# Shridhar2602/WebGPU-Path-Tracer

Hardware: AMD Instinct MI355X
Metric: Mrays/s at 1080p, 8 bounces; achieved HBM GB/s vs roofline (higher is better)
Workload: dtype f32; 1 GPU; configs[1]: Cornell + monkey_968.obj (967 tris), 1920x1080, 64 spp, 8 bounces, stack_size 20; parallelism=1 GPU

## Files before the change

webgpu-path-tracer_amd/csrc/ptmi.hip:

```cpp
#include <dlfcn.h>
#include <hip/hip_runtime.h>
#include <rccl/rccl.h>

#include <algorithm>
#include <chrono>
#include <cmath>
#include <cstdio>
#include <cstdlib>
#include <condition_variable>
#include <cstring>
#include <functional>
#include <map>
#include <memory>
#include <mutex>
#include <string>
#include <thread>
#include <type_traits>
#include <vector>

#include "../../include/ptmi.h"
#include "ptmi_dbuf.h"
#include "ptmi_kernels.h"
#include "ptmi_denoise_kernels.h"
#include "ptmi_tuning.h"
// ... 705 lines not shown
    HIP_TRY(c, hipEventRecord(ev.e0, c->stream));
    if (int r = dry()) return r;
    HIP_TRY(c, hipEventRecord(ev.e1, c->stream));
    HIP_TRY(c, hipEventSynchronize(ev.e1));
    HIP_TRY(c, hipEventElapsedTime(ms, ev.e0, ev.e1));
    return PTMI_OK;
  };
  float best = 0.0f;
  if (int r = score(&best)) return r;
  uint64_t sets = 1;
  if (c->tun.debug_placement) fprintf(stderr, "ptmi placement: set 0 %.3f ms\n", best);
  DBuf* mine[10] = {&c->d_q0[0], &c->d_q0[1], &c->d_q1[0], &c->d_q1[1], &c->d_q2[0], &c->d_q2[1], &c->d_tp[0], &c->d_tp[1], &c->d_hm[0], &c->d_hm[1]};
  const size_t width[10] = {16, 16, 16, 16, 16, 16, 8, 8, 4, 4};
  int rc_out = PTMI_OK;
  std::vector<DBuf> losers;
  size_t set_bytes = 0;
  for (int k = 0; k < 10; k++) set_bytes += slots * width[k];
  for (int t = 1; t < c->tun.placement_tries; t++) {
    size_t mem_free = 0, mem_total = 0;
    if (hipMemGetInfo(&mem_free, &mem_total) != hipSuccess) mem_free = 0, (void)hipGetLastError();
    if (mem_free < set_bytes + ((size_t)8 << 30)) {
      if (losers.empty()) break;
      losers.clear();
    }
    DBuf cand[10];
    bool ok = true;
    for (int k = 0; k < 10 && ok; k++) ok = cand[k].ensure(slots * width[k]) == hipSuccess;
    float ms = 0.0f;
    if (ok) {
      for (int k = 0; k < 10; k++) std::swap(*mine[k], cand[k]);
      rc_out = score(&ms);
      ok = rc_out == PTMI_OK;
      if (ok) sets++;
      if (c->tun.debug_placement) fprintf(stderr, "ptmi placement: set %d %.3f ms\n", t, ms);
      if (!ok || ms >= best) {
        for (int k = 0; k < 10; k++) std::swap(*mine[k], cand[k]);
      } else {
        best = ms;
      }
    }
    if (!ok) {
      (void)hipStreamSynchronize(c->stream);
      break;
    }
    for (DBuf& b : cand)
      if (b.p) losers.push_back(std::move(b));
  }
  restore.stats.placement_sets = sets;
  restore.stats.placement_ms = std::chrono::duration<double, std::milli>(std::chrono::steady_clock::now() - t_search).count();
  return rc_out;
}

RenderConst make_render_const(const ptmi_ctx* c, const float* view16, uint32_t frame0, int n_frames, int reset_first) {
  const ptmi_params& p = c->prm;
  RenderConst rc{};
  rc.W = (float)c->W;
  rc.H = (float)c->H;
  memcpy(rc.view, view16, 64);
  {
    const float* m = rc.view;
    for (int k = 0; k < 3; k++) rc.cam_o[k] = ((m[k] * 0.0f + m[4 + k] * 0.0f) + m[8 + k] * 0.0f) + m[12 + k] * 1.0f;
  }
  rc.fov_factor = (float)(1.0 / std::tan((double)p.fov_degrees * (3.14159265358979323846 / 180.0) / 2.0));
  rc.bg[0] = p.background[0], rc.bg[1] = p.background[1], rc.bg[2] = p.background[2];
  rc.max_bounces = p.max_bounces;
  rc.stratify = p.stratify ? 1 : 0;
  if (p.stratify) {
    float sqrt_spp = (float)std::sqrt((double)p.num_samples);
    int side = 0;
    for (float i = 0.0f; i < sqrt_spp; i += 1.0f) side++;
    rc.strat_side = side;
    rc.recip_sqrt_spp = 1.0f / (float)(int)sqrt_spp;
    rc.num_samples = side * side;
    rc.sample_div = (float)(side * side);
  } else {
    rc.strat_side = 1;
    rc.recip_sqrt_spp = 1.0f;
    rc.num_samples = p.num_samples;
    rc.sample_div = (float)p.num_samples;
  }
  rc.stack_size = p.stack_size;
  rc.light_mix = p.light_mix;
  rc.surface_mix = 1.0f - p.light_mix;
  rc.npix = (uint32_t)c->W * (uint32_t)c->H;
  rc.frame0 = frame0;
  rc.n_frames = n_frames;
  rc.reset_first = reset_first;
  rc.rank = c->rank, rc.world = c->world, rc.tile = c->tile;
  rc.n_local = count_local(rc.npix, c->rank, c->world, c->tile);
  rc.shade_cont = (uint32_t)c->tun.shade_cont;
  return rc;
}

struct ViewBatch {
  ViewTab vt;
  float4* stack;
};

int render_batch(ptmi_ctx* c, const float* view16, uint32_t frame0, int n_frames, int reset_first, int fold = -1, int dry_steps = 0, const ViewBatch* views = nullptr) {
  const ptmi_params& p = c->prm;
  c->ahead.valid = false;
  const RenderConst rc = make_render_const(c, view16, frame0, n_frames, reset_first);
  if (rc.n_local == 0) return PTMI_OK;
  ViewTab vtab{};
  if (views) vtab = views->vt, vtab.n_local = rc.n_local;
  const ViewTab* vt = views ? &vtab : nullptr;

  const int n_steps = rc.num_samples * p.max_bounces;
  const size_t npaths = (size_t)rc.n_local * (size_t)n_frames;
  c->batch_enqueued = false;
  int rcode = ensure_paths(c, npaths, n_steps + 2, rc.num_samples > 1);
  if (rcode) return rcode;
  StepCtl* ctl = c->d_ctl.as<StepCtl>();
  const uint32_t total = rc.n_local * (uint32_t)n_frames;
  const int sa_carry = stack_alloc_for(c);
  const bool carry = c->tun.bvh_carry > 0 && c->S.n_nodes > 0 && c->bvh_depth >= c->tun.bvh_carry_min_depth && total >= (uint32_t)c->tun.bvh_carry_min_paths && p.max_bounces > 1;
  const uint32_t resv = carry ? (uint32_t)c->tun.bvh_carry_slots : 0u;
  const int rec_words = carry_rec_words(sa_carry);
  if (carry)
    for (int k = 0; k < 2; k++) HIP_TRY(c, c->d_carry[k].ensure((size_t)resv * (size_t)rec_words * 4));
  auto carry_of = [&](int s) {
    Carry cy{};
    cy.resv = s == 0 ? 0u : resv;
    cy.resv_next = resv;
    cy.after = c->tun.bvh_carry;
    cy.rec_words = rec_words;
    cy.pool_in = c->d_carry[s & 1].as<uint32_t>();
    cy.pool_out = c->d_carry[(s + 1) & 1].as<uint32_t>();
    return cy;
  };
  const uint32_t bound = total + total / 8 + (uint32_t)c->num_cus * 8 * 1024 + resv;
  const uint32_t ew_grid = std::max<uint32_t>(1, std::min<uint32_t>((total + kBlock - 1) / kBlock, (uint32_t)c->num_cus * 16));
  const int sort_env = c->tun.sort;
  const bool sort = sort_env >= 0 ? sort_env != 0 : c->material_classes > 1;

  const auto shade = with_flags([](auto is, auto so, auto cn, auto mu) { return shade_kernel<is, so, cn, mu>(); }, p.importance_sampling != 0, sort, c->counters,
                                rc.num_samples > 1);
  const auto shade_views = with_flags([](auto is, auto so, auto cn, auto mu) { return shade_views_kernel<is, so, cn, mu>(); }, p.importance_sampling != 0, sort, c->counters,
                                      rc.num_samples > 1);
  int shade_bpc = c->tun.shade_blocks_per_cu;
  if (shade_bpc <= 0) {
    int& cached = c->shade_blocks_per_cu[views ? reinterpret_cast<const void*>(shade_views) : reinterpret_cast<const void*>(shade)];
    if (cached == 0) {
      int nb = 0;
      const hipError_t oe = views ? hipOccupancyMaxActiveBlocksPerMultiprocessor(&nb, shade_views, kBlock, 0) : hipOccupancyMaxActiveBlocksPerMultiprocessor(&nb, shade, kBlock, 0);
      if (oe != hipSuccess || nb < 1) nb = 5;
      cached = nb;
    }
    shade_bpc = cached;
  }
  const uint32_t sgrid = std::max<uint32_t>(1, std::min<uint32_t>((bound + kSChunk - 1) / kSChunk, (uint32_t)c->num_cus * (uint32_t)std::min(8, std::max(1, shade_bpc))));
  unsigned long long* tot = c->d_totals.as<unsigned long long>();
  const TailPlan tail = tail_plan(c, rc);

  if (dry_steps == 0 && c->placement_pending) {
    c->placement_pending = false;
    if (total > tail.limit_first) {
      int r = placement_search(c, [&]() { return render_batch(c, view16, frame0, n_frames, reset_first, fold, 2, views); });
      if (r) return r;
    }
  }
  ScopedSpan whole(c, T_RENDER);
  c->batch_enqueued = true;
  hipLaunchKernelGGL(k_init_ctl, dim3((unsigned)((n_steps + 2 + 63) / 64)), dim3(64), 0, c->stream, ctl, n_steps + 2, resv);
  HIP_TRY(c, hipMemsetAsync(tot + 16, 0, kTotalsBytes - 128, c->stream));
  {
    ScopedSpan s(c, T_GENERATE);
    if (rc.num_samples == 1) HIP_TRY(c, hipMemsetAsync(c->d_touched.p, 0, npaths, c->stream));
    if (views) {
      const auto generate = with_flags([](auto cn) { return &k_generate_views<cn>; }, c->counters);
      hipLaunchKernelGGL(generate, dim3(ew_grid), dim3(kBlock), 0, c->stream, c->S, rc, paths_of(c, 0, rc.num_samples > 1), ctl, c->d_heads.as<uint32_t>(), tot, vtab);
    } else {
      const auto generate = with_flags([](auto cn) { return &k_generate<cn>; }, c->counters);
      hipLaunchKernelGGL(generate, dim3(ew_grid), dim3(kBlock), 0, c->stream, c->S, rc, paths_of(c, 0, rc.num_samples > 1), ctl, c->d_heads.as<uint32_t>(), tot);
    }
    HIP_TRY(c, hipGetLastError());
    c->stats.generate_launches++;
  }
  bool drained = false;
  const int run_steps = dry_steps > 0 ? std::min(n_steps, dry_steps) : n_steps;
  for (int s = 0; s < run_steps; s++) {
    if (s >= 12 && (s & 7) == 4) {
      uint32_t left = 1;
      uint32_t rec3[3] = {1, 0, 0};
      HIP_TRY(c, hipMemcpyAsync(rec3, &ctl[s].n_rays, sizeof rec3, hipMemcpyDeviceToHost, c->stream));
      HIP_TRY(c, hipStreamSynchronize(c->stream));
      left = (rec3[0] <= resv && rec3[2] == 0) ? 0u : 1u;
      if (left == 0) {
        drained = true;
        break;
      }
    }
    Paths P = paths_of(c, s, rc.num_samples > 1);
    if (const uint32_t tail_limit = dry_steps > 0 ? 0u : (s == 0 ? tail.limit_first : tail.limit_later)) {
      int lr = launch_tail(c, rc, P, ctl + s, s == 0 ? 1 : 0, tail_limit, tail.six, carry_of(s), vt);
      if (lr) return lr;
      if (s == 0 && total <= tail_limit) {
        drained = true;
        break;
      }
    }
    if (dry_steps == 0) {
      Carry cy = carry_of(s);
      if (!carry || s >= n_steps - c->tun.bvh_carry_last) cy.resv_next = 0u;
      int lr = launch_intersect(c, P, ctl + s, bound, false, s == 0 ? &rc : nullptr, cy, vt);
      if (lr) return lr;
    }
    {
      ScopedSpan sp(c, T_SHADE);
      if (views) hipLaunchKernelGGL(shade_views, dim3(sgrid), dim3(kBlock), 0, c->stream, c->S, rc, P, ctl + s, c->d_heads.as<uint32_t>(), tot, s == 0 ? 1 : 0, s == 0 ? 0u : resv, vtab);
      else hipLaunchKernelGGL(shade, dim3(sgrid), dim3(kBlock), 0, c->stream, c->S, rc, P, ctl + s, c->d_heads.as<uint32_t>(), tot, s == 0 ? 1 : 0, s == 0 ? 0u : resv);
      HIP_TRY(c, hipGetLastError());
    }
    c->stats.intersect_launches++;
    c->stats.shade_launches++;
  }
  if (dry_steps > 0) return PTMI_OK;
  if (carry && !drained && n_steps > 0) {
    int lr = launch_tail(c, rc, paths_of(c, n_steps, rc.num_samples > 1), ctl + n_steps, 0, 0xffffffffu, tail.six, carry_of(n_steps), vt);
    if (lr) return lr;
  }
  {
    ScopedSpan s(c, T_ACCUM);
    const int f_end = fold < 0 ? n_frames : std::min(fold, n_frames);
    if (views) hipLaunchKernelGGL(k_accumulate<true>, dim3(ew_grid), dim3(kBlock), 0, c->stream, rc, paths_of(c, 0, rc.num_samples > 1), views->stack, n_steps, tot, 0, f_end, vtab);
    else hipLaunchKernelGGL(k_accumulate<false>, dim3(ew_grid), dim3(kBlock), 0, c->stream, rc, paths_of(c, 0, rc.num_samples > 1), c->fb, n_steps, tot, 0, f_end, vtab);
    c->stats.accumulate_launches++;
  }
  HIP_TRY(c, hipGetLastError());
  c->stats.frames += (uint64_t)n_frames;
  c->ahead.rc = rc;
  c->ahead.grid = ew_grid;
  return PTMI_OK;
}

int check_queue_overflow(ptmi_ctx* c) {
  if (!c->d_totals.p) return PTMI_OK;
  unsigned long long flag = 0;
  HIP_TRY(c, hipMemcpy(&flag, c->d_totals.as<unsigned long long>() + 15, sizeof flag, hipMemcpyDeviceToHost));
  if (flag) return fail(c, PTMI_ERR_STATE, "internal: a step's queue outgrew its buffer (paths were dropped); the framebuffer is incomplete");
  return PTMI_OK;
}

int check_renderable(ptmi_ctx* c) {
  if (!c->fb || c->W <= 0) return fail(c, PTMI_ERR_STATE, "no framebuffer: call ptmi_resize first");
  const ptmi_params& p = c->prm;
  if (p.importance_sampling && c->has_unknown_material)
    return fail(c, PTMI_ERR_UNSUPPORTED,
                "importance_sampling with a material_type outside {0,1,2,3}: the shader would read stale private state (scatterRec)");
  return PTMI_OK;
}

struct Rccl {
  void* lib = nullptr;
  decltype(&ncclCommInitAll) CommInitAll = nullptr;
  decltype(&ncclCommDestroy) CommDestroy = nullptr;
  decltype(&ncclCommAbort) CommAbort = nullptr;
  decltype(&ncclReduce) Reduce = nullptr;
  decltype(&ncclGroupStart) GroupStart = nullptr;
  decltype(&ncclGroupEnd) GroupEnd = nullptr;
  decltype(&ncclGetErrorString) GetErrorString = nullptr;
  std::string why;
  bool load() {
    if (lib) return true;
    const char* names[] = {getenv("PTMI_RCCL_LIB"), "librccl.so.1", "librccl.so", "/opt/rocm/lib/librccl.so.1"};
    for (const char* n : names) {
      if (!n || !*n) continue;
      lib = dlopen(n, RTLD_NOW | RTLD_LOCAL);
      if (lib) break;
      why = dlerror();
    }
    if (!lib) return false;
#define PTMI_RCCL_SYM(field, sym)                                  \
  field = reinterpret_cast<decltype(field)>(dlsym(lib, #sym));     \
  if (!field) {                                                    \
    why = std::string("librccl lacks ") + #sym;                    \
    dlclose(lib);                                                  \
    lib = nullptr;                                                 \
    return false;                                                  \
  }
    PTMI_RCCL_SYM(CommInitAll, ncclCommInitAll)
    PTMI_RCCL_SYM(CommDestroy, ncclCommDestroy)
    PTMI_RCCL_SYM(CommAbort, ncclCommAbort)
    PTMI_RCCL_SYM(Reduce, ncclReduce)
    PTMI_RCCL_SYM(GroupStart, ncclGroupStart)
    PTMI_RCCL_SYM(GroupEnd, ncclGroupEnd)
    PTMI_RCCL_SYM(GetErrorString, ncclGetErrorString)
#undef PTMI_RCCL_SYM
    return true;
  }
};
Rccl g_rccl;
inline int rccl_fail_hook(const ptmi_ctx* c) {
#ifdef PTMI_TEST_HOOKS
  return c->test_rccl_fail;
#else
  (void)c;
  return 0;
#endif
}
std::once_flag g_rccl_once;
bool rccl_loaded() {
  std::call_once(g_rccl_once, [] { (void)g_rccl.load(); });
  return g_rccl.lib != nullptr;
}

#define RCCL_TRY(c, expr)                                                                                            \
  do {                                                                                                               \
    ncclResult_t _r = (expr);                                                                                        \
    if (_r != ncclSuccess) return fail((c), PTMI_ERR_DEVICE, std::string(#expr) + ": " + g_rccl.GetErrorString(_r)); \
  } while (0)

template <class F>
int on_all_devices(ptmi_ctx* c, F fn, bool parallel = false) {
  const std::vector<ptmi_ctx*> devs = local_devices(c);
  std::vector<int> rcs(devs.size(), PTMI_OK);
  if (parallel) {
    for (ptmi_ctx* q : c->peers) {
      if (!q->worker) q->worker = std::make_unique<PeerWorker>();
      q->worker->post([&fn, q] { return fn(q); });
    }
    rcs[0] = fn(c);
    for (size_t i = 1; i < devs.size(); i++) rcs[i] = devs[i]->worker->wait();
  } else {
    for (size_t i = 0; i < devs.size(); i++)
      if ((rcs[i] = fn(devs[i]))) break;
  }
  for (size_t i = 1; i < devs.size(); i++)
    if (rcs[i] && !rcs[0]) {
      c->err = "local device #" + std::to_string(i) + " (GPU " + std::to_string(devs[i]->device) + "): " + devs[i]->err;
      return rcs[i];
    }
  return rcs[0];
}

__global__ __launch_bounds__(kBlock) void k_gather_tiles(float4* __restrict__ dst, const float4* __restrict__ src, uint32_t n_local, int rank, int world, int tile) {
  for (uint32_t j = blockIdx.x * kBlock + threadIdx.x; j < n_local; j += gridDim.x * kBlock) {
    const uint32_t tl = j / (uint32_t)tile, within = j - tl * (uint32_t)tile;
    const uint32_t pix = (tl * (uint32_t)world + (uint32_t)rank) * (uint32_t)tile + within;
    dst[pix] = src[pix];
  }
}

__global__ __launch_bounds__(kBlock) void k_add_into(float4* __restrict__ dst, const float4* __restrict__ src, size_t n) {
  for (size_t i = (size_t)blockIdx.x * kBlock + threadIdx.x; i < n; i += (size_t)gridDim.x * kBlock) {
    const float4 a = dst[i], b = src[i];
    dst[i] = make_float4(a.x + b.x, a.y + b.y, a.z + b.z, a.w + b.w);
// ... 1327 lines not shown
```

webgpu-path-tracer_amd/csrc/ptmi_kernels.h:

```cpp
#pragma once
#include "ptmi_device.h"
#include "ptmi_tuning.h"

namespace ptmi {

constexpr int kBlock = 256;

DEV void reset_heads(uint32_t* __restrict__ heads) {
  if (blockIdx.x == 0 && threadIdx.x < kMaxTeams) heads[threadIdx.x * kHeadStride] = 0u;
}

DEV void reduce_counters(const Counters& cn, unsigned long long* __restrict__ totals, bool bvh) {
  uint32_t v[5] = {cn.node_visits, cn.tri_tests, cn.sphere_tests, cn.quad_tests, cn.mat_fetches};
#pragma unroll
  for (int k = 0; k < 5; k++) {
    unsigned long long x = v[k];
    for (int off2 = 32; off2 > 0; off2 >>= 1) x += __shfl_down(x, off2, 64);
    if (lane_id() == 0 && x) {
      atomicAdd(&totals[2 + k], x);
      if (bvh && k == 0) atomicAdd(&totals[7], x);
      if (bvh && k == 4) atomicAdd(&totals[8], x);
    }
  }
}
// ... 477 lines not shown
        float pdf = rc.light_mix * lpdf + rc.surface_mix * lambertian_pdf;
        if (pdf <= 0.00001f) {
          drop_acc = true;
          sample_done = true;
        } else {
          T = T * ((lambertian_pdf * mix3(m.color, m.spec, doSpecular)) / pdf);
          no = so;
          nd = sd;
        }
      }
    } else {
      T = T * mix3(m.color, m.spec, doSpecular);
      no = sorg;
      nd = sdir;
    }
    if (!sample_done) {
      if (roulette && bounce > 2) {
        LT(LT_RR);
        float p = ptm_max(T.x, ptm_max(T.y, T.z));
        if (rand2D(rng) > p) {
          sample_done = true;
        } else {
          T = T * rcp_exact(p);
        }
      }
      if (!sample_done) {
        bounce++;
        if (bounce >= rc.max_bounces) sample_done = true;
      }
    }
  }

  const bool changes = !(add.x == 0.0f && add.y == 0.0f && add.z == 0.0f);
  ns.pid = pid;
  if (!sample_done) {
    if (changes) {
      LT(LT_ACC_CONT);
      float4 A4 = acc_load(P, pid, acc_written);
      f3 acc = mk3(A4) + add;
      acc_store(P, pid, make_float4(acc.x, acc.y, acc.z, A4.w), acc_written);
      acc_written = true;
    }
    ns.o = no, ns.d = nd, ns.T = T, ns.bounce = bounce | (acc_written ? kAccWritten : 0), ns.rng = rng;
    return true;
  }

  LT(LT_END_SAMPLE);
  if (!MULTI) {
    if (drop_acc) {
      f3 fin = mk3(0, 0, 0) + add;
      acc_store(P, pid, make_float4(fin.x, fin.y, fin.z, __int_as_float(1)), acc_written);
    } else {
      end_sample_progressive(P, pid, add, acc_written);
    }
    return false;
  } else {
  float4 A4 = P.acc[pid];
  int sample = __float_as_int(A4.w);
  f3 radiance = drop_acc ? add : (mk3(A4) + add);
  f3 sum = mk3(P.pixsum[pid]) + radiance;
  sample++;
  if (sample < rc.num_samples) {
    P.pixsum[pid] = make_float4(sum.x, sum.y, sum.z, 0.0f);
    if (MV) camera_ray_view(rc, vt, pid, sample, rng, no, nd);
    else camera_ray(rc, local_to_pixel(rc, pid % rc.n_local), sample, rng, no, nd);
    P.acc[pid] = make_float4(0.0f, 0.0f, 0.0f, __int_as_float(sample));
    ns.o = no, ns.d = nd, ns.T = mk3(1.0f, 1.0f, 1.0f), ns.bounce = 0, ns.rng = rng;
    return true;
  }
  f3 fin = sum / rc.sample_div;
  P.acc[pid] = make_float4(fin.x, fin.y, fin.z, __int_as_float(sample));
  return false;
  }
}

constexpr uint32_t kRegionDiv = 16;
constexpr uint32_t kRegionDivCont = 64;
constexpr int kTailLimitFirst = 2 << 20, kTailLimitLater = 1 << 20;
constexpr int kTailLimitFirstShallow = 24 << 20, kTailLimitLaterShallow = 2 << 20;
constexpr int kTailLimitFirstDeep = 6 << 20;
constexpr int kTailRefill = 16;
constexpr bool kMissShortcut = true;
constexpr int kSChunk = 512;

constexpr uint32_t kR0Empty = 0xffffffffu, kR0Busy = 0xfffffffeu, kR0Full = 0xfffffffdu;
__shared__ uint32_t s_region0;
constexpr uint32_t kNoSlot = 0xffffffffu;
struct OutRegion {
  uint32_t cur, rend;
  DEV uint32_t place(bool keep, uint32_t region, uint32_t wregion, uint32_t wregion_later, StepCtl* __restrict__ ctl, uint32_t cap, unsigned long long* __restrict__ totals) {
    const int lane = lane_id();
    const uint64_t km = __ballot(keep);
    const uint32_t kept = (uint32_t)__popcll(km), rank = lanes_below(km);
    const uint32_t b0 = cur, n0 = min(kept, rend - cur);
    uint32_t b1 = kNoSlot;
    cur += n0;
    if (kept > n0) {
      uint32_t nb = 0, claimed = wregion;
      bool full;
      if (rend == 0u) {
        if (lane == 0) nb = atomicCAS(&s_region0, kR0Empty, kR0Busy);
        nb = (uint32_t)__builtin_amdgcn_readfirstlane((int)nb);
        if (nb == kR0Empty) {
          if (lane == 0) {
            nb = atomicAdd(&ctl[1].n_rays, region);
            if (nb + region > cap) {
              atomicAdd(&totals[15], 1ull);
              atomicSub(&ctl[1].n_rays, region);
              nb = kR0Full;
            }
            atomicExch(&s_region0, nb);
          }
          nb = (uint32_t)__builtin_amdgcn_readfirstlane((int)nb);
        } else {
          while (nb == kR0Busy) {
            __builtin_amdgcn_s_sleep(8);
            if (lane == 0) nb = atomicAdd(&s_region0, 0u);
            nb = (uint32_t)__builtin_amdgcn_readfirstlane((int)nb);
          }
        }
        full = nb == kR0Full;
        nb += (threadIdx.x >> 6) * wregion;
      } else {
        claimed = wregion_later;
        if (lane == 0) nb = atomicAdd(&ctl[1].n_rays, claimed);
        nb = (uint32_t)__builtin_amdgcn_readfirstlane((int)nb);
        full = nb + claimed > cap;
        if (full && lane == 0) {
          atomicAdd(&totals[15], 1ull);
          atomicSub(&ctl[1].n_rays, claimed);
        }
      }
      if (!full) {
        b1 = nb;
        cur = nb + (kept - n0);
        rend = nb + claimed;
      }
    }
    if (keep && (rank < n0 || b1 != kNoSlot)) return (rank < n0) ? (b0 + rank) : (b1 + (rank - n0));
    return kNoSlot;
  }
  DEV void close(const Paths& P, uint32_t wregion, bool block_claim) {
    if (rend == 0u && block_claim && s_region0 < kR0Full) {
      cur = s_region0 + (threadIdx.x >> 6) * wregion;
      rend = cur + wregion;
    }
    for (uint32_t i = cur + (uint32_t)lane_id(); i < rend; i += 64u) {
      LT(LT_HOLE);
      mark_hole(P.out, P.hout, i);
    }
  }
};

template <bool IS, bool COUNT, bool MULTI, bool MV>
DEV void shade_body(const DevScene& S, const RenderConst& rc, const Paths& P, StepCtl* __restrict__ ctl, uint32_t* __restrict__ heads, unsigned long long* __restrict__ totals,
                    int first, uint32_t resv, const ViewTab& vt) {
  reset_heads(heads);
  __shared__ float4 s_q0[kSChunk], s_q1[kSChunk], s_q2[kSChunk];
  __shared__ uint16_t s_sorted[kSChunk];
  __shared__ uint32_t s_cnt[NUM_BINS + 2];
  __shared__ uint32_t s_nout, s_next;
  const QuadL L = load_light(S);
  const int lane = lane_id();
  const QueueExtent qe = queue_extent(ctl, resv);
  const uint32_t n = qe.n, n_carried = qe.n_carried;
  const uint32_t region = max((uint32_t)kSChunk, ((n / gridDim.x / kRegionDiv) + 511u) & ~511u);
  const uint32_t wregion = region / (kBlock / 64);
  OutRegion out = {0u, 0u};
  if (threadIdx.x == 0) s_region0 = kR0Empty;
  uint32_t my_valid = 0;
  uint32_t my_missed = 0;
  Counters cn = {0, 0, 0, 0, 0};
  auto stage = [&](bool survive, const NewState& ns) {
    const uint64_t mk = __ballot(survive);
    if (mk) {
      const int leader = __ffsll((unsigned long long)mk) - 1;
      uint32_t bb = 0;
      if (lane == leader) bb = atomicAdd(&s_nout, (uint32_t)__popcll(mk));
      bb = (uint32_t)__shfl((int)bb, leader, 64);
      if (survive) {
        const uint32_t q = bb + lanes_below(mk);
        s_q0[q] = pack_q0(ns);
        s_q1[q] = pack_q1(ns);
        s_q2[q] = pack_q2(ns);
      }
    }
  };
  for (uint32_t base = blockIdx.x * (uint32_t)kSChunk; base < n; base += gridDim.x * (uint32_t)kSChunk) {
    const uint32_t m = min((uint32_t)kSChunk, n - base);
    if (threadIdx.x < NUM_BINS) s_cnt[threadIdx.x] = 0;
    if (threadIdx.x == 0) {
      s_nout = 0;
      s_next = 0;
    }
    __syncthreads();
    {
      uint32_t keys[kSChunk / kBlock];
      uint32_t words[kSChunk / kBlock];
  #pragma unroll
      for (int r = 0; r < kSChunk / kBlock; r++) words[r] = P.hin.mat[base + min((uint32_t)r * kBlock + threadIdx.x, m - 1u)];
  #pragma unroll
      for (int r = 0; r < kSChunk / kBlock; r++) {
        const uint32_t j = (uint32_t)r * kBlock + threadIdx.x;
        int bin = -1;
        if (j < m && !dead_slot(base + j, n_carried, resv)) {
          const uint32_t b = (words[r] >> HITMAT_BIN_SHIFT) & 7u;
          if (b < (uint32_t)NUM_BINS) bin = (int)b;
        }
        uint32_t rank = 0;
        if ((uint32_t)r * kBlock < m) rank = bin_rank(bin, s_cnt);
        keys[r] = (bin < 0) ? 0xffffffffu : ((uint32_t)bin | (rank << 3));
      }
      __syncthreads();
      uint32_t nvalid = 0;
      {
        uint32_t off[NUM_BINS];
  #pragma unroll
        for (int b = 0; b < NUM_BINS; b++) {
          off[b] = nvalid;
          nvalid += s_cnt[b];
        }
  #pragma unroll
        for (int r = 0; r < kSChunk / kBlock; r++) {
          if (keys[r] != 0xffffffffu) {
            const uint32_t b = keys[r] & 7u;
            uint32_t o = off[0];
  #pragma unroll
            for (int k = 1; k < NUM_BINS; k++) o = (b == (uint32_t)k) ? off[k] : o;
            s_sorted[o + (keys[r] >> 3)] = (uint16_t)((uint32_t)r * kBlock + threadIdx.x);
          }
        }
      }
      if (threadIdx.x == 0) my_valid += nvalid;
      __syncthreads();
#pragma unroll 1
      for (;;) {
        uint32_t k0 = 0;
        if (lane == 0) k0 = atomicAdd(&s_next, 64u);
        k0 = (uint32_t)__builtin_amdgcn_readfirstlane((int)k0);
        if (k0 >= nvalid) break;
        const uint32_t k = k0 + lane;
        bool survive = false;
        NewState ns = zero_state();
        if (k < nvalid) {
          const SlotState st = load_slot<MV>(P, base + s_sorted[k], first != 0, rc, vt);
          const TriFetch tf = tri_fetch(S, P.uv, st.slot, __float_as_uint(st.tp.y));
          survive = shade_one<IS, MULTI, MV>(S, rc, P, st, tf, L, ns, vt);
        }
        stage(survive, ns);
      }
    }
    __syncthreads();
    const uint32_t cnt = s_nout;
    uint32_t missed = 0;
#pragma unroll 1
    for (uint32_t q0 = (threadIdx.x & ~63u); q0 < cnt; q0 += kBlock) {
      const uint32_t q = q0 + (uint32_t)lane;
      bool keep = false;
      float2 tp = make_float2(0.0f, 0.0f);
      uint32_t hm = 0u, rng = 0u;
      if (q < cnt) {
        const float4 a0 = s_q0[q], a1 = s_q1[q];
        rng = __float_as_uint(a0.w);
        prims_for_ray<COUNT>(S, mk3(a0), mk3(a1), rng, tp, hm, cn);
        if (kMissShortcut && !MULTI && hm == HITMAT_MISS) {
          const float4 a2 = s_q2[q];
          end_sample_progressive(P, __float_as_uint(a1.w), mk3(rc.bg[0], rc.bg[1], rc.bg[2]) * mk3(a2), (__float_as_int(a2.w) & kAccWritten) != 0);
          missed++;
        } else {
          keep = true;
        }
      }
      if (__ballot(keep) == 0ull) continue;
      const uint32_t dst = out.place(keep, region, wregion, wregion, ctl, P.cap, totals);
      if (dst != kNoSlot) {
        float4 a0 = s_q0[q];
        a0.w = __uint_as_float(rng);
        store_slot(P.out, P.hout, dst, a0, s_q1[q], s_q2[q], tp, hm);
      }
    }
    if (!MULTI) {
      for (int off2 = 32; off2 > 0; off2 >>= 1) missed += __shfl_down(missed, off2, 64);
      if (lane == 0) my_missed += missed;
    }
    __syncthreads();
  }
  if (lane == 0 && my_missed + my_valid) atomicAdd(tally_line(totals, blockIdx.x), my_missed + my_valid);
  out.close(P, wregion, blockIdx.x * (uint32_t)kSChunk < n);
  if (COUNT) reduce_counters(cn, totals, false);
}

template <bool IS, bool COUNT, bool MULTI, bool MV>
DEV void shade_body_wave(const DevScene& S, const RenderConst& rc, const Paths& P, StepCtl* __restrict__ ctl, uint32_t* __restrict__ heads,
                         unsigned long long* __restrict__ totals, int first, uint32_t resv, const ViewTab& vt) {
  reset_heads(heads);
  constexpr uint32_t kRing = 128, kWaves = kBlock / 64;
  static_assert((size_t)kWaves * kRing == (size_t)kSChunk, "the rings take the LDS the block version's staging arrays take");
  __shared__ float4 s_q0[kWaves * kRing], s_q1[kWaves * kRing], s_q2[kWaves * kRing];
  if (threadIdx.x == 0) s_region0 = kR0Empty;
#ifdef PTMI_LANE_TALLY
  if (threadIdx.x < kLaneTallies * 2) s_lane_tally[threadIdx.x] = 0u;
  if (threadIdx.x < 4 * kTimeTallies) s_time_tally[threadIdx.x] = 0ull;
  if (threadIdx.x < 4) s_time_last[threadIdx.x] = 0ull;
#endif
  __syncthreads();
  const QuadL L = load_light(S);
  const int lane = lane_id();
  const uint32_t wv = threadIdx.x >> 6;
  float4 *const r0 = s_q0 + wv * kRing, *const r1 = s_q1 + wv * kRing, *const r2 = s_q2 + wv * kRing;
  const QueueExtent qe = queue_extent(ctl, resv);
  const uint32_t n = qe.n, n_carried = qe.n_carried;
  const uint32_t cont_min = MULTI ? 0u : rc.shade_cont;
  const uint32_t region_full = max((uint32_t)kSChunk, ((n / gridDim.x / kRegionDiv) + 511u) & ~511u);
  const uint32_t region = cont_min ? max((uint32_t)kSChunk, ((n / gridDim.x / kRegionDivCont) + 511u) & ~511u) : region_full;
  const uint32_t wregion = region / kWaves, wregion_full = region_full / kWaves;
  bool pred = true;
  OutRegion out = {0u, 0u};
  uint32_t head = 0, cnt = 0;
  uint32_t my_valid = 0, my_missed = 0;
  Counters cn = {0, 0, 0, 0, 0};
  auto flush_pass = [&](uint32_t take, SlotState& cs, bool cont) {
    const uint32_t q = (head + (uint32_t)lane) & (kRing - 1u);
    bool keep = false;
    float2 tp = make_float2(0.0f, 0.0f);
    uint32_t hm = 0u, rng = 0u;
    if ((uint32_t)lane < take) {
      LT(LT_FLUSH);
      const float4 a0 = r0[q], a1 = r1[q];
      TT(TT_RING_READ, a0.x + a1.x);
      rng = __float_as_uint(a0.w);
      prims_for_ray<COUNT>(S, mk3(a0), mk3(a1), rng, tp, hm, cn);
      TT(TT_FLUSH_PRIMS, tp.x + __uint_as_float(hm));
      if (kMissShortcut && !MULTI && hm == HITMAT_MISS) {
        LT(LT_MISS_SHORTCUT);
        const float4 a2 = r2[q];
        end_sample_progressive(P, __float_as_uint(a1.w), mk3(rc.bg[0], rc.bg[1], rc.bg[2]) * mk3(a2), (__float_as_int(a2.w) & kAccWritten) != 0);
      } else {
        keep = true;
      }
    }
    bool go = false;
    if (cont_min) {
      const bool final_hit = keep && (hm & HITMAT_BVH) == 0u;
      pred = (uint32_t)__popcll(__ballot(final_hit)) >= cont_min;
      if (cont && pred) {
        go = final_hit;
        keep = keep && !final_hit;
      }
    }
    const uint64_t km = __ballot(keep);
    const uint32_t kept = (uint32_t)__popcll(km);
    my_missed += take - kept - (uint32_t)__popcll(__ballot(go));
    if (kept) {
      const uint32_t dst = out.place(keep, region, wregion, pred ? wregion : wregion_full, ctl, P.cap, totals);
      if (dst != kNoSlot) {
        LT(LT_KEEP);
        float4 a0 = r0[q];
        a0.w = __uint_as_float(rng);
        store_slot(P.out, P.hout, dst, a0, r1[q], r2[q], tp, hm);
      }
    }
    if (cont) {
      if (go) LT(LT_CONT);
      cs.q0 = r0[q];
      cs.q0.w = __uint_as_float(rng);
      cs.q1 = r1[q];
      cs.q2 = r2[q];
      cs.tp = tp;
      cs.hitmat = hm;
      cs.slot = 0u;
    }
    head = (head + take) & (kRing - 1u);
    cnt -= take;
    TT(TT_FLUSH_STORE, 0.0f);
    return go;
  };
  auto shade_group = [&](bool active, const SlotState& st) {
    bool survive = false, valid = false;
    NewState ns = zero_state();
    TT(TT_OTHER, 0.0f);
    if (active) {
      LT(LT_GROUP);
      TT(TT_LOAD1, st.q0.x + st.q1.x + st.q2.x + st.tp.x + __uint_as_float(st.hitmat));
      valid = __float_as_uint(st.q1.w) != PID_HOLE;
      if (valid) {
        LT(LT_VALID);
        const TriFetch tf = tri_fetch(S, P.uv, st.slot, __float_as_uint(st.tp.y));
        survive = shade_one<IS, MULTI, MV>(S, rc, P, st, tf, L, ns, vt);
      }
    }
    TT(TT_SHADE, ns.o.x + ns.T.x);
    my_valid += (uint32_t)__popcll(__ballot(valid));
    const uint64_t mk = __ballot(survive);
    if (survive) {
      LT(LT_STAGE);
      const uint32_t q = (head + cnt + lanes_below(mk)) & (kRing - 1u);
      r0[q] = pack_q0(ns);
      r1[q] = pack_q1(ns);
      r2[q] = pack_q2(ns);
    }
    cnt += (uint32_t)__popcll(mk);
    TT(TT_STAGE, 0.0f);
  };
  {
    uint32_t base = blockIdx.x * (uint32_t)kSChunk, j0 = wv * 64u;
    auto settle = [&]() {
      while (base < n && j0 >= min((uint32_t)kSChunk, n - base)) {
        base += gridDim.x * (uint32_t)kSChunk;
        j0 = wv * 64u;
      }
      return base < n;
    };
    auto fetch = [&](SlotState& st) {
      const uint32_t j = j0 + (uint32_t)lane;
      const bool act = j < min((uint32_t)kSChunk, n - base) && !dead_slot(base + j, n_carried, resv);
      if (act) st = load_slot<MV>(P, base + j, first != 0, rc, vt);
      return act;
    };
    SlotState cur;
    bool have = settle(), cur_act = false, again = false;
    if (have) cur_act = fetch(cur);
#pragma unroll 1
    while (have || again) {
      shade_group(cur_act, cur);
      if (!again) {
        j0 += kBlock;
        have = settle();
      }
      const bool flush_due = cnt >= 64u;
      const bool pre = have && !(cont_min && flush_due && pred);
      SlotState nxt;
      bool nxt_act = false;
      if (pre) nxt_act = fetch(nxt);
      bool go = false;
      if (flush_due) go = flush_pass(64u, nxt, cont_min != 0u && !pre);
      again = __ballot(go) != 0ull;
      if (again) nxt_act = go;
      else if (have && !pre) nxt_act = fetch(nxt);
      cur = nxt;
      cur_act = nxt_act;
    }
    if (cnt) flush_pass(cnt, cur, false);
  }
  if (MULTI) my_missed = 0;
  if (lane == 0 && my_missed + my_valid) atomicAdd(tally_line(totals, blockIdx.x), my_missed + my_valid);
  __syncthreads();
#ifdef PTMI_LANE_TALLY
  if (threadIdx.x < kLaneTallies * 2 && s_lane_tally[threadIdx.x]) atomicAdd(&g_lane_tally[threadIdx.x], (unsigned long long)s_lane_tally[threadIdx.x]);
  if (threadIdx.x < kTimeTallies) {
    unsigned long long t = 0;
    for (int w = 0; w < 4; w++) t += s_time_tally[w * kTimeTallies + threadIdx.x];
    if (t) atomicAdd(&g_time_tally[threadIdx.x], t);
  }
#endif
  out.close(P, wregion, true);
#ifdef PTMI_LANE_TALLY
  __syncthreads();
  if (threadIdx.x >= 2 * LT_HOLE && threadIdx.x < 2 * LT_HOLE + 2 && s_lane_tally[threadIdx.x]) atomicAdd(&g_lane_tally[threadIdx.x], (unsigned long long)s_lane_tally[threadIdx.x]);
#endif
  if (COUNT) reduce_counters(cn, totals, false);
}

template <bool IS, bool SORT, bool COUNT, bool MULTI>
__global__ __launch_bounds__(kBlock) PTMI_SHADE_ATTR void k_shade(DevScene S, RenderConst rc, Paths P, StepCtl* __restrict__ ctl, uint32_t* __restrict__ heads,
                                                                  unsigned long long* __restrict__ totals, int first, uint32_t resv) {
  if constexpr (SORT) shade_body<IS, COUNT, MULTI, false>(S, rc, P, ctl, heads, totals, first, resv, ViewTab{});
  else shade_body_wave<IS, COUNT, MULTI, false>(S, rc, P, ctl, heads, totals, first, resv, ViewTab{});
}
template <bool SORT, bool COUNT>
__global__ __launch_bounds__(kBlock) __attribute__((amdgpu_waves_per_eu(6, 8))) void k_shade6(DevScene S, RenderConst rc, Paths P, StepCtl* __restrict__ ctl,
                                                                                                uint32_t* __restrict__ heads, unsigned long long* __restrict__ totals, int first, uint32_t resv) {
  if constexpr (SORT) shade_body<false, COUNT, false, false>(S, rc, P, ctl, heads, totals, first, resv, ViewTab{});
  else shade_body_wave<false, COUNT, false, false>(S, rc, P, ctl, heads, totals, first, resv, ViewTab{});
}
template <bool IS, bool SORT, bool COUNT, bool MULTI>
__global__ __launch_bounds__(kBlock) PTMI_SHADE_ATTR void k_shade_views(DevScene S, RenderConst rc, Paths P, StepCtl* __restrict__ ctl, uint32_t* __restrict__ heads,
                                                                        unsigned long long* __restrict__ totals, int first, uint32_t resv, ViewTab vt) {
  if constexpr (SORT) shade_body<IS, COUNT, MULTI, true>(S, rc, P, ctl, heads, totals, first, resv, vt);
  else shade_body_wave<IS, COUNT, MULTI, true>(S, rc, P, ctl, heads, totals, first, resv, vt);
}
template <bool SORT, bool COUNT>
__global__ __launch_bounds__(kBlock) __attribute__((amdgpu_waves_per_eu(6, 8))) void k_shade6_views(DevScene S, RenderConst rc, Paths P, StepCtl* __restrict__ ctl,
                                                                                                      uint32_t* __restrict__ heads, unsigned long long* __restrict__ totals, int first,
                                                                                                      uint32_t resv, ViewTab vt) {
  if constexpr (SORT) shade_body<false, COUNT, false, true>(S, rc, P, ctl, heads, totals, first, resv, vt);
  else shade_body_wave<false, COUNT, false, true>(S, rc, P, ctl, heads, totals, first, resv, vt);
}

constexpr int kTailTravBatch = 24;
template <bool IS, bool COUNT, bool MULTI, bool NOABORT, bool MV>
DEV void tail_body(const DevScene& S, const RenderConst& rc, const Paths& P, StepCtl* __restrict__ ctl, unsigned long long* __restrict__ totals, int first, uint32_t limit,
                   int stack_size, int lds_entries, int spill_entries, int2* __restrict__ spill, const Carry& cy, const ViewTab& vt) {
  const QueueExtent qe = queue_extent(ctl, cy.resv);
  const uint32_t n = qe.n, n_carried = qe.n_carried;
  if (n == 0u) return;
  if ((n > cy.resv ? n - cy.resv : 0u) + n_carried > limit) return;
  extern __shared__ int lds_stack[];
  const int lane = lane_id();
  LaneStack2 stk;
  stk.lds = (lds_v2i_t*)lds_stack + lane;
  stk.spill = spill + (size_t)blockIdx.x * (size_t)spill_entries * 64 + lane;
  stk.lds_entries = lds_entries;
  const QuadL L = load_light(S);
  Counters cn = {0, 0, 0, 0, 0}, cb = {0, 0, 0, 0, 0};
  uint32_t tally = 0;
  const uint32_t root = __float_as_uint(S.root_lo.w);
  const uint32_t root_node = (root & REF_LEAF) ? root : (root & REF_IDX);
  SlotState st;
  st.q0 = st.q1 = st.q2 = make_float4(0.0f, 0.0f, 0.0f, 0.0f);
  st.tp = make_float2(0.0f, 0.0f);
  st.hitmat = HITMAT_HOLE, st.slot = 0;
  bool alive = false;
  bool resume = false;
  int park_sp = -1;
  float2 uv = make_float2(0.0f, 0.0f);
  uint32_t gnext = blockIdx.x, gbase = 0, pos = 64;
  Stopwatch sw;
  sw.begin();
#pragma unroll 1
  for (;;) {
    BT(TB_VOTE, 0.0f, 0);
    uint64_t am = __ballot(alive);
    const uint32_t nidle = 64u - (uint32_t)__popcll(am);
    if (nidle >= (uint32_t)kTailRefill || am == 0ull) {
      if (pos == 64u && gnext * 64u < n) {
        gbase = gnext * 64u;
        gnext += gridDim.x;
        pos = 0;
      }
      if (pos < 64u) {
        const uint32_t take = min(nidle, 64u - pos), rank = lanes_below(~am);
        if (!alive && rank < take) {
          const uint32_t slot = gbase + pos + rank;
          if (slot < n && !dead_slot(slot, n_carried, cy.resv)) {
            st = load_slot<MV>(P, slot, first != 0, rc, vt);
            alive = __float_as_uint(st.q1.w) != PID_HOLE;
            uv = make_float2(0.0f, 0.0f);
            resume = alive && slot < cy.resv;
          }
        }
        pos += take;
        am = __ballot(alive);
        BT(TB_TAKE, st.q1.x + st.tp.x + __uint_as_float(st.hitmat), take);
      }
    }
    if (am == 0ull) {
      if (pos == 64u && gnext * 64u >= n) break;
      continue;
    }
    {
      const bool flagged = alive && (st.hitmat & HITMAT_BVH) != 0u;
      const uint64_t fmask = __ballot(flagged);
      const bool more_to_take = !(pos == 64u && gnext * 64u >= n);
      if (fmask != 0ull && ((int)__popcll(fmask) >= (more_to_take ? kTailTravBatch : 1) || __ballot(alive && !flagged) == 0ull)) {
        Walk w = {flagged ? root_node : N_DONE, 0, st.tp.x, {0.0f, 0.0f, 0u, 0u}};
        WalkRay ray = make_walk_ray(S, mk3(st.q0), mk3(st.q1));
        if (flagged && resume) carry_restore(cy, st.slot, stk, w);
        resume = false;
        if (flagged && park_sp >= 0) {
          unpark(stk, park_sp, w);
          park_sp = -1;
        }
#pragma unroll 1
        for (;;) {
          const uint64_t wm = __ballot(w.node != N_DONE);
          if (wm == 0ull) break;
          if (cy.park_below > 0 && (int)__popcll(wm) < cy.park_below && (more_to_take || __ballot(alive && !(flagged && w.node != N_DONE)) != 0ull)) break;
          if ((int)w.node < 0) {
            walk_leaf<COUNT>(S, ray, stk, w, cb, sw);
            BT(TB_WALK_LEAF, w.ct, __popcll(__ballot(1)));
          }
          if (w.node < N_INNER_LIMIT) walk_inner<COUNT, NOABORT, TB_WALK_FETCH>(S, ray, stk, w, stack_size, cb, sw);
          BT(TB_WALK_STEP, __uint_as_float(w.node), __popcll(__ballot(w.node != N_DONE)));
        }
        if (flagged && w.node != N_DONE) {
          park(stk, w);
          park_sp = w.sp;
        } else {
          if (w.hit.prim != 0u) {
            st.tp = make_float2(w.ct, __uint_as_float(w.hit.prim));
            uv = make_float2(w.hit.u, w.hit.v);
            st.hitmat = w.hit.mat;
          }
          st.hitmat &= ~HITMAT_BVH;
        }
      }
      const bool go = alive && (st.hitmat & HITMAT_BVH) == 0u;
      NewState ns = zero_state();
      bool survive = false;
      if (go) {
        tally++;
        const TriFetch tf = tri_fetch_uv(S, uv, __float_as_uint(st.tp.y));
        survive = shade_one<IS, MULTI, MV>(S, rc, P, st, tf, L, ns, vt);
        alive = survive;
      }
      BT(TB_SHADE, ns.o.x + ns.T.x, __popcll(__ballot(go)));
      if (go && alive) {
        uint32_t hm;
        float2 tp;
        prims_for_ray<COUNT>(S, ns.o, ns.d, ns.rng, tp, hm, cn);
        if (kMissShortcut && !MULTI && hm == HITMAT_MISS) {
          end_sample_progressive(P, ns.pid, mk3(rc.bg[0], rc.bg[1], rc.bg[2]) * ns.T, (ns.bounce & kAccWritten) != 0);
          tally++;
          alive = false;
        } else {
          st.q0 = pack_q0(ns);
          st.q1 = pack_q1(ns);
          st.q2 = pack_q2(ns);
          st.tp = tp;
          st.hitmat = hm;
        }
      }
      BT(TB_PRIMS, st.tp.x, __popcll(__ballot(go && survive)));
    }
  }
  BT_FLUSH(g_tail_tally);
  for (int off2 = 32; off2 > 0; off2 >>= 1) tally += __shfl_down(tally, off2, 64);
  if (lane == 0 && tally) atomicAdd(tally_line(totals, blockIdx.x), tally);
  if (COUNT) {
    reduce_counters(cn, totals, false);
    reduce_counters(cb, totals, true);
  }
  if (lane == 0) {
    __threadfence();
    if (atomicAdd(&ctl->tail_done, 1u) == gridDim.x - 1u) {
      ctl->n_rays = 0u;
// ... 334 lines not shown
```

Baseline: 29500 Mrays/s.

## Fuse camera ray generation with first-bounce shading in a persistent kernel

Adds a generating variant of the wave-level shade kernel that creates camera rays, intersects them, and shades first hits in place, writing surviving paths into the input queue through per-wave regions. It is used in progressive single-view, non-sorted mode when the camera lies outside the scene root box, and it skips the separate first-step tail launch. The aim is to avoid writing primary rays to memory and reading them back in a separate generate pass. In exchange the host code picks between two generate paths, the fused kernel carries more register pressure, and each wave emits holes for unused queue slots.

```diff
diff --git a/webgpu-path-tracer_amd/csrc/ptmi.hip b/webgpu-path-tracer_amd/csrc/ptmi.hip
--- a/webgpu-path-tracer_amd/csrc/ptmi.hip
+++ b/webgpu-path-tracer_amd/csrc/ptmi.hip
@@ -881,6 +881,27 @@
   const uint32_t sgrid = std::max<uint32_t>(1, std::min<uint32_t>((bound + kSChunk - 1) / kSChunk, (uint32_t)c->num_cus * (uint32_t)std::min(8, std::max(1, shade_bpc))));
   unsigned long long* tot = c->d_totals.as<unsigned long long>();
   const TailPlan tail = tail_plan(c, rc);
+  bool cam_in_root = c->S.n_nodes > 0;
+  {
+    const float lo[3] = {c->S.root_lo.x, c->S.root_lo.y, c->S.root_lo.z}, hi[3] = {c->S.root_hi.x, c->S.root_hi.y, c->S.root_hi.z};
+    for (int k = 0; k < 3; k++) cam_in_root = cam_in_root && rc.cam_o[k] >= lo[k] && rc.cam_o[k] <= hi[k];
+  }
+  const bool fused = rc.num_samples == 1 && !sort && c->tun.shade_cont > 0 && !views && total > tail.limit_first && !cam_in_root;
+  const auto generate_shade = with_flags([](auto cn, auto is) { return &k_generate<cn, is>; }, c->counters, p.importance_sampling != 0);
+  uint32_t ggrid = ew_grid;
+  if (fused) {
+    int bpc = c->tun.shade_blocks_per_cu;
+    if (bpc <= 0) {
+      int& cached = c->shade_blocks_per_cu[reinterpret_cast<const void*>(generate_shade)];
+      if (cached == 0) {
+        int nb = 0;
+        if (hipOccupancyMaxActiveBlocksPerMultiprocessor(&nb, generate_shade, kBlock, 0) != hipSuccess || nb < 1) nb = 5;
+        cached = nb;
+      }
+      bpc = cached;
+    }
+    ggrid = std::max<uint32_t>(1, std::min<uint32_t>((total + kSChunk - 1) / kSChunk, (uint32_t)c->num_cus * (uint32_t)std::min(8, std::max(1, bpc))));
+  }
 
   if (dry_steps == 0 && c->placement_pending) {
     c->placement_pending = false;
@@ -899,6 +920,8 @@
     if (views) {
       const auto generate = with_flags([](auto cn) { return &k_generate_views<cn>; }, c->counters);
       hipLaunchKernelGGL(generate, dim3(ew_grid), dim3(kBlock), 0, c->stream, c->S, rc, paths_of(c, 0, rc.num_samples > 1), ctl, c->d_heads.as<uint32_t>(), tot, vtab);
+    } else if (fused) {
+      hipLaunchKernelGGL(generate_shade, dim3(ggrid), dim3(kBlock), 0, c->stream, c->S, rc, paths_of(c, 0, false), ctl, c->d_heads.as<uint32_t>(), tot);
     } else {
       const auto generate = with_flags([](auto cn) { return &k_generate<cn>; }, c->counters);
       hipLaunchKernelGGL(generate, dim3(ew_grid), dim3(kBlock), 0, c->stream, c->S, rc, paths_of(c, 0, rc.num_samples > 1), ctl, c->d_heads.as<uint32_t>(), tot);
@@ -921,7 +944,7 @@
       }
     }
     Paths P = paths_of(c, s, rc.num_samples > 1);
-    if (const uint32_t tail_limit = dry_steps > 0 ? 0u : (s == 0 ? tail.limit_first : tail.limit_later)) {
+    if (const uint32_t tail_limit = dry_steps > 0 ? 0u : (s == 0 ? (fused ? 0u : tail.limit_first) : tail.limit_later)) {
       int lr = launch_tail(c, rc, P, ctl + s, s == 0 ? 1 : 0, tail_limit, tail.six, carry_of(s), vt);
       if (lr) return lr;
       if (s == 0 && total <= tail_limit) {
diff --git a/webgpu-path-tracer_amd/csrc/ptmi_kernels.h b/webgpu-path-tracer_amd/csrc/ptmi_kernels.h
--- a/webgpu-path-tracer_amd/csrc/ptmi_kernels.h
+++ b/webgpu-path-tracer_amd/csrc/ptmi_kernels.h
@@ -653,6 +653,46 @@
   }
 };
 
+DEV float fresh_s(float x) {
+  asm volatile("" : "+s"(x));
+  return x;
+}
+DEV uint32_t fresh_s(uint32_t x) {
+  asm volatile("" : "+s"(x));
+  return x;
+}
+struct GenRegion {
+  uint32_t cur, rend;
+  DEV uint32_t place(bool keep, uint32_t wregion, StepCtl* __restrict__ ctl, uint32_t cap, unsigned long long* __restrict__ totals) {
+    const int lane = lane_id();
+    const uint64_t km = __ballot(keep);
+    const uint32_t kept = (uint32_t)__popcll(km), rank = lanes_below(km);
+    const uint32_t b0 = cur, n0 = min(kept, rend - cur);
+    uint32_t b1 = kNoSlot;
+    cur += n0;
+    if (kept > n0) {
+      uint32_t nb = 0;
+      if (lane == 0) nb = atomicAdd(&ctl[0].n_rays, wregion);
+      nb = (uint32_t)__builtin_amdgcn_readfirstlane((int)nb);
+      const bool full = nb + wregion > cap;
+      if (full && lane == 0) {
+        atomicAdd(&totals[15], 1ull);
+        atomicSub(&ctl[0].n_rays, wregion);
+      }
+      if (!full) {
+        b1 = nb;
+        cur = nb + (kept - n0);
+        rend = nb + wregion;
+      }
+    }
+    if (keep && (rank < n0 || b1 != kNoSlot)) return (rank < n0) ? (b0 + rank) : (b1 + (rank - n0));
+    return kNoSlot;
+  }
+  DEV void close(const Paths& P) {
+    for (uint32_t i = cur + (uint32_t)lane_id(); i < rend; i += 64u) mark_hole(P.in, P.hin, i);
+  }
+};
+
 template <bool IS, bool COUNT, bool MULTI, bool MV>
 DEV void shade_body(const DevScene& S, const RenderConst& rc, const Paths& P, StepCtl* __restrict__ ctl, uint32_t* __restrict__ heads, unsigned long long* __restrict__ totals,
                     int first, uint32_t resv, const ViewTab& vt) {
@@ -791,10 +831,12 @@
   if (COUNT) reduce_counters(cn, totals, false);
 }
 
-template <bool IS, bool COUNT, bool MULTI, bool MV>
+template <bool IS, bool COUNT, bool MULTI, bool MV, bool GEN = false>
 DEV void shade_body_wave(const DevScene& S, const RenderConst& rc, const Paths& P, StepCtl* __restrict__ ctl, uint32_t* __restrict__ heads,
                          unsigned long long* __restrict__ totals, int first, uint32_t resv, const ViewTab& vt) {
+  static_assert(!GEN || (!MULTI && !MV), "the generating instance: progressive mode, one view");
   reset_heads(heads);
+  if (GEN && rc.max_bounces <= 0) return;
   constexpr uint32_t kRing = 128, kWaves = kBlock / 64;
   static_assert((size_t)kWaves * kRing == (size_t)kSChunk, "the rings take the LDS the block version's staging arrays take");
   __shared__ float4 s_q0[kWaves * kRing], s_q1[kWaves * kRing], s_q2[kWaves * kRing];
@@ -809,7 +851,7 @@
   const int lane = lane_id();
   const uint32_t wv = threadIdx.x >> 6;
   float4 *const r0 = s_q0 + wv * kRing, *const r1 = s_q1 + wv * kRing, *const r2 = s_q2 + wv * kRing;
-  const QueueExtent qe = queue_extent(ctl, resv);
+  const QueueExtent qe = GEN ? QueueExtent{rc.n_local * (uint32_t)rc.n_frames, 0u} : queue_extent(ctl, resv);
   const uint32_t n = qe.n, n_carried = qe.n_carried;
   const uint32_t cont_min = MULTI ? 0u : rc.shade_cont;
   const uint32_t region_full = max((uint32_t)kSChunk, ((n / gridDim.x / kRegionDiv) + 511u) & ~511u);
@@ -853,7 +895,7 @@
     const uint32_t kept = (uint32_t)__popcll(km);
     my_missed += take - kept - (uint32_t)__popcll(__ballot(go));
     if (kept) {
-      const uint32_t dst = out.place(keep, region, wregion, pred ? wregion : wregion_full, ctl, P.cap, totals);
+      const uint32_t dst = out.place(keep, region, wregion, (GEN || pred) ? wregion : wregion_full, ctl, P.cap, totals);
       if (dst != kNoSlot) {
         LT(LT_KEEP);
         float4 a0 = r0[q];
@@ -903,7 +945,82 @@
     cnt += (uint32_t)__popcll(mk);
     TT(TT_STAGE, 0.0f);
   };
-  {
+  if constexpr (GEN) {
+    const uint32_t groups = (rc.n_local + 63u) / 64u, n_waves = gridDim.x * kWaves;
+    const uint32_t step_f = n_waves / groups, step_g = n_waves - step_f * groups;
+    const uint32_t wregion0 = max(64u, ((n / n_waves / 16u) + 63u) & ~63u);
+    GenRegion in0 = {0u, 0u};
+    auto generate = [&](uint32_t f, uint32_t g, SlotState& st) {
+      const uint32_t j = g * 64u + (uint32_t)lane;
+      bool keep = false;
+      float2 tp = make_float2(0.0f, 0.0f);
+      uint32_t hm = 0u, rng = 0u, pid = 0u;
+      RenderConst cr = rc;
+      cr.W = fresh_s(rc.W);
+      cr.fov_factor = fresh_s(rc.fov_factor);
+      cr.tile = (int)fresh_s((uint32_t)rc.tile);
+#pragma unroll
+      for (int k = 0; k < 16; k++) cr.view[k] = fresh_s(rc.view[k]);
+#pragma unroll
+      for (int k = 0; k < 3; k++) cr.cam_o[k] = fresh_s(rc.cam_o[k]);
+      f3 o = cam_origin(cr), d = mk3(0, 0, 0);
+      const bool mine = j < rc.n_local;
+      if (mine) {
+        const uint32_t pix = local_to_pixel(cr, j);
+        float px, py;
+        camera_pixel(cr, pix, px, py);
+        pid = f * rc.n_local + j;
+        rng = pix + (uint32_t)(float)(rc.frame0 + f) * 719393u;
+        camera_ray_at(cr, px, py, 0, rng, o, d);
+        prims_for_ray<COUNT>(S, o, d, rng, tp, hm, cn);
+        if (kMissShortcut && hm == HITMAT_MISS) {
+          end_sample_progressive(P, pid, mk3(rc.bg[0], rc.bg[1], rc.bg[2]) * mk3(1.0f, 1.0f, 1.0f), false);
+        } else {
+          keep = true;
+        }
+      }
+      const bool final_hit = keep && (hm & HITMAT_BVH) == 0u;
+      const bool act = cont_min != 0u && (uint32_t)__popcll(__ballot(final_hit)) >= cont_min && final_hit;
+      const bool store = keep && !act;
+      my_missed += (uint32_t)__popcll(__ballot(mine && !keep));
+      if (__ballot(store) != 0ull) {
+        const uint32_t dst = in0.place(store, wregion0, ctl, P.cap, totals);
+        if (dst != kNoSlot) {
+          rng0_of(P)[dst] = rng;
+          P.in.q1[dst] = make_float4(d.x, d.y, d.z, __uint_as_float(pid));
+          P.hin.tp[dst] = tp;
+          P.hin.mat[dst] = hm;
+        }
+      }
+      st.q0 = make_float4(o.x, o.y, o.z, __uint_as_float(rng));
+      st.q1 = make_float4(d.x, d.y, d.z, __uint_as_float(pid));
+      st.q2 = make_float4(1.0f, 1.0f, 1.0f, __int_as_float(0));
+      st.tp = tp;
+      st.hitmat = hm;
+      st.slot = 0u;
+      return act;
+    };
+    SlotState cur;
+    bool cur_act = false, again = false;
+    const uint32_t w0 = blockIdx.x * kWaves + wv;
+    uint32_t f = w0 / groups, g = w0 - f * groups;
+#pragma unroll 1
+    while (f < (uint32_t)rc.n_frames || again) {
+      if (!again) {
+        cur_act = generate(f, g, cur);
+        f += step_f, g += step_g;
+        if (g >= groups) g -= groups, f++;
+      }
+      again = false;
+      if (__ballot(cur_act) != 0ull) shade_group(cur_act, cur);
+      if (cnt >= 64u) {
+        cur_act = flush_pass(64u, cur, cont_min != 0u);
+        again = __ballot(cur_act) != 0ull;
+      }
+    }
+    if (cnt) flush_pass(cnt, cur, false);
+    in0.close(P);
+  } else {
     uint32_t base = blockIdx.x * (uint32_t)kSChunk, j0 = wv * 64u;
     auto settle = [&]() {
       while (base < n && j0 >= min((uint32_t)kSChunk, n - base)) {
@@ -973,6 +1090,11 @@
                                                                                                 uint32_t* __restrict__ heads, unsigned long long* __restrict__ totals, int first, uint32_t resv) {
   if constexpr (SORT) shade_body<false, COUNT, false, false>(S, rc, P, ctl, heads, totals, first, resv, ViewTab{});
   else shade_body_wave<false, COUNT, false, false>(S, rc, P, ctl, heads, totals, first, resv, ViewTab{});
+}
+template <bool COUNT, bool IS>
+__global__ __launch_bounds__(kBlock) __attribute__((amdgpu_waves_per_eu(IS ? 5 : 6, 8))) void k_generate(DevScene S, RenderConst rc, Paths P, StepCtl* __restrict__ ctl,
+                                                                                                           uint32_t* __restrict__ heads, unsigned long long* __restrict__ totals) {
+  shade_body_wave<IS, COUNT, false, false, true>(S, rc, P, ctl, heads, totals, 1, 0u, ViewTab{});
 }
 template <bool IS, bool SORT, bool COUNT, bool MULTI>
 __global__ __launch_bounds__(kBlock) PTMI_SHADE_ATTR void k_shade_views(DevScene S, RenderConst rc, Paths P, StepCtl* __restrict__ ctl, uint32_t* __restrict__ heads,
```

New measurement: 28570 Mrays/s. 3.2% lower.
